# wq2012/SpectralCluster

Measured on AMD Instinct MI355X. Metric: predict() calls/sec, n=8192 d=256 ICASSP2018 (GraphCut, eigengap k in [2,20], cosine k-means), higher is better.
Workload: dtype f64; 1 GPU; icassp2018_graphcut_n8192_d256_k8_max20; n_samples=8192, n_features=256, parallelism=replicas x1, collectives=none

## Files before the change

### include/spectralcluster_amd.h

```cpp
#ifndef SPECTRALCLUSTER_AMD_H_
#define SPECTRALCLUSTER_AMD_H_

#include <stddef.h>
#include <stdint.h>

#ifdef __cplusplus
extern "C" {
#endif

#define SC_ABI_VERSION 8
#define SC_MAX_OPS 16
#define SC_MAX_BLUR_RADIUS 32
#define SC_MAX_EIG 128
#define SC_MAX_STAGES 16

typedef struct sc_handle_s* sc_handle;

typedef enum sc_status {
  SC_OK = 0,
  SC_ERR_INVALID = -1,
  SC_ERR_OOM = -2,
  SC_ERR_HIP = -3,
  SC_ERR_NOT_CONVERGED = -4,
  SC_ERR_UNSUPPORTED = -5,
// ... 231 lines not shown
                                   const double* const* affinities, const double* const* bands,
                                   double* const* outs);
int sc_stage_diffuse_rowstats(sc_handle h, const double* a, int n, int mode, double* rowmax,
                              double* rowsum, int32_t* info);
enum {
  SC_BLOCK_ROUTE_SYM = 1,
  SC_BLOCK_ROUTE_TWO_PRODUCT = 2,
  SC_BLOCK_ROUTE_GROUPED = 4
};
int sc_stage_block_operator(sc_handle h, int count, const int32_t* ns,
                            const double* const* matrices, const double* const* cvecs,
                            const double* const* pvecs, const double* const* vs_scales,
                            const double* const* vs, double* const* ws, int route);
int sc_stage_krylov_state(sc_handle h, int32_t* info, double* q, double* t, double* g, double* c,
                          double* p);
int sc_stage_laplacian(sc_handle h, int laplacian_type, const double* in, int n,
                       double* out);
int sc_stage_sym_eig(sc_handle h, const double* m, int n, int count, int descend,
                     double* values, double* vectors, sc_diag* diag);
int sc_stage_eig(sc_handle h, const double* m, int n, int count, int descend,
                 double* values, double* vectors, sc_diag* diag);
int sc_random_state_doubles(uint32_t seed, int count, double* out);
int sc_uniform_choice(int n, double u);
int sc_host_symmetric_eig(const double* a, int m, double* values, double* vectors);
int sc_host_symmetric_eig_partial(const double* a, int m, int need, double* values,
                                  double* vectors);
int sc_host_tridiag_eigvectors(const double* d, const double* e, int n, const double* lam,
                               int k, double* vectors);
int sc_host_general_eig(const double* a, int m, int nvec, double* values_re, double* values_im,
                        double* vectors_re, double* vectors_im);
// ... 40 lines not shown
```

### spectralcluster_amd/_lib.py

```python

from __future__ import annotations

import ctypes
import os
import threading
import typing

import numpy as np

SC_MAX_OPS = 16
SC_MAX_BLUR_RADIUS = 32
SC_MAX_EIG = 128
SC_MAX_STAGES = 16

SC_OK = 0
SC_ERR_INVALID = -1
SC_ERR_OOM = -2
SC_ERR_HIP = -3
SC_ERR_NOT_CONVERGED = -4
SC_ERR_UNSUPPORTED = -5
SC_ERR_NON_FINITE = -6

STAGE_NAMES = ("affinity", "refine", "diffuse", "scaling", "eig", "kmeans",
               "total", "blur", "threshold_sym", "matvec", "affinity_gemm",
# ... 127 lines not shown
    "sc_set_free_prune": (ctypes.c_int, [_handle_t, ctypes.c_int]),
    "sc_stage_diffuse_rowstats": (ctypes.c_int, [_handle_t, _c_double_p, ctypes.c_int,
                                                 ctypes.c_int, _c_double_p, _c_double_p,
                                                 ctypes.POINTER(ctypes.c_int32)]),
    "sc_stage_block_operator": (ctypes.c_int, [_handle_t, ctypes.c_int,
                                               ctypes.POINTER(ctypes.c_int32),
                                               ctypes.POINTER(_c_double_p),
                                               ctypes.POINTER(_c_double_p),
                                               ctypes.POINTER(_c_double_p),
                                               ctypes.POINTER(_c_double_p),
                                               ctypes.POINTER(_c_double_p),
                                               ctypes.POINTER(_c_double_p), ctypes.c_int]),
    "sc_stage_krylov_state": (ctypes.c_int, [_handle_t, ctypes.POINTER(ctypes.c_int32),
                                             _c_double_p, _c_double_p, _c_double_p, _c_double_p,
                                             _c_double_p]),
    "sc_config_default": (ctypes.c_int, [ctypes.POINTER(ScConfig)]),
    "sc_gaussian_weights": (ctypes.c_int, [ctypes.c_double,
                                           ctypes.POINTER(ctypes.c_int32),
                                           _c_double_p]),
    "sc_predict": (ctypes.c_int, [_handle_t, _c_double_p, ctypes.c_int, ctypes.c_int,
                                  ctypes.POINTER(ScConfig), _c_int64_p,
                                  ctypes.POINTER(ScDiag)]),
    "sc_set_embeddings": (ctypes.c_int, [_handle_t, _c_double_p, ctypes.c_int,
                                         ctypes.c_int]),
    "sc_predict_array": (ctypes.c_int, [_handle_t, ctypes.POINTER(ScArray),
                                        ctypes.POINTER(ScConfig), _c_int64_p,
                                        ctypes.POINTER(ScDiag)]),
    "sc_set_embeddings_array": (ctypes.c_int, [_handle_t, ctypes.POINTER(ScArray)]),
    "sc_predict_batch_arrays": (ctypes.c_int, [_handle_t, ctypes.POINTER(ScArray), ctypes.c_int,
                                               ctypes.POINTER(ScConfig),
# ... 336 lines not shown
```

### spectralcluster_amd/csrc/api.hip

```cpp
#include <algorithm>
#include <array>
#include <cmath>
#include <cstdio>
#include <cstdlib>
#include <cstring>
#include <vector>

#include <condition_variable>
#include <mutex>
#include <string>
#include <thread>

#include "handle.h"
#include "host_pool.h"

int ensure_matrices(sc_handle h, int n, int d, bool affinity_copy) {
  h->krylov_m = 0;
  const size_t ldn = matrix_ld(n);
  const size_t nn = (size_t)n * ldn * sizeof(double);
  if (affinity_copy) SC_TRY(grow(h, h->A0, nn));
  SC_TRY(grow(h, h->B1, nn));
  SC_TRY(grow(h, h->B2, nn));
  if (d > 0) {
    const size_t ldx = round_up(d, 16);
// ... 33 lines not shown
      SC_HIP(h, hipStreamSynchronize(h->stream));
    }
    h->tilemap_cur = ptr<int2>(h->tilemap_table) + h->tilemap_off[nt];
    return SC_OK;
  }
  if (h->tilemap_nt != nt) {
    std::vector<int2> map;
    gemm_build_sym_tilemap(nt, &map);
    SC_TRY(grow(h, h->tilemap, map.size() * sizeof(int2)));
    SC_HIP(h, hipMemcpyAsync(h->tilemap.p, map.data(), map.size() * sizeof(int2),
                             hipMemcpyHostToDevice, h->stream));
    SC_HIP(h, hipStreamSynchronize(h->stream));
    h->tilemap_nt = nt;
  }
  h->tilemap_cur = ptr<int2>(h->tilemap);
  return SC_OK;
}

int ensure_eig(sc_handle h, int n) {
  const size_t nq = (size_t)n * kLdq * sizeof(double);
  if (h->Q.bytes < nq) h->krylov_m = 0;
  SC_TRY(grow(h, h->Q, nq));
  SC_TRY(grow(h, h->Q2, nq));
  SC_TRY(grow(h, h->Vs, (size_t)n * kEigBlock * sizeof(double)));
  SC_TRY(grow(h, h->W, (size_t)n * kEigBlock * sizeof(double)));
  SC_TRY(grow(h, h->partial, std::max((size_t)kProjBlocks * kLdq * kEigBlock,
                                       lz_partial_doubles(n)) * sizeof(double)));
  SC_TRY(grow(h, h->T, (size_t)kLdq * kLdq * sizeof(double)));
  SC_TRY(grow(h, h->Y, (size_t)kLdq * kLdq * sizeof(double)));
  SC_TRY(grow(h, h->Yt, (size_t)kLdq * kLdq * sizeof(double)));
// ... 98 lines not shown
  h->pool.clear();
  for (sc_handle sub : h->gslots) sc_destroy(sub);
  h->gslots.clear();
  for (sc_handle sub : h->gshort) sc_destroy(sub);
  h->gshort.clear();
  hipSetDevice(h->device);
  hipStreamSynchronize(h->stream);
  DevBuf* bufs[] = {&h->X,     &h->Xn,    &h->A0,     &h->B1,      &h->B2,    &h->rowmax,
                    &h->rowsum, &h->cvec,  &h->pvec,   &h->tvec,    &h->deg,   &h->blurw, &h->blur_tmp, &h->dvec, &h->cut, &h->rmpart, &h->splitk, &h->tilemap, &h->tilemap_table, &h->cropval, &h->statp, &h->crvec, &h->thetai, &h->Vre, &h->Vim, &h->gpart, &h->gsrc, &h->genL, &h->ahc_size, &h->ahc_chain, &h->ahc_Z, &h->ahc_lab, &h->ahc_cent, &h->fb_part, &h->fb_small, &h->fb_x, &h->fb_cent, &h->fb_int, &h->Cq, &h->Cband, &h->cp[0], &h->cp[1], &h->cp[2], &h->cp[3], &h->cp[4], &h->symflag,
                    &h->Q,     &h->Q2,    &h->Vs,     &h->W,       &h->partial, &h->T,
                    &h->Y,     &h->Yt,    &h->theta,  &h->resid,   &h->G,     &h->Rinv,
                    &h->Hbuf,  &h->hsq,   &h->colnorm, &h->flags,  &h->E,     &h->Ek,   &h->Eio,
                    &h->td_d,  &h->td_e,  &h->td_theta, &h->td_work, &h->td_tau, &h->td_panel, &h->mvsym,
                    &h->kXc,   &h->kxsq,  &h->kclosest, &h->kcand, &h->kenorm, &h->krnd,
                    &h->kcent, &h->klab32, &h->klab64, &h->kinfo, &h->kchain, &h->gkrnd, &h->gpack, &h->gypack, &h->ginfo, &h->glabels, &h->gjtab,
                    &h->kbig, &h->kbigw, &h->fq, &h->ft32, &h->fy1, &h->fR, &h->fscal, &h->fwords, &h->fcand, &h->fY, &h->fsplit, &h->fypart, &h->frpart, &h->fq2part, &h->fmx64, &h->ftau64, &h->fplan, &h->Xalt, &h->Xstage, &h->gneg};
  for (DevBuf* b : bufs)
    if (b->p) hipFree(b->p);
  for (DevBuf& b : h->kgen)
    if (b.p) hipFree(b.p);
  for (int i = 0; i < 48; ++i) hipEventDestroy(h->ev[i]);
  if (h->h_theta) hipHostFree(h->h_theta);
  if (h->h_flags) hipHostFree(h->h_flags);
  if (h->h_rr) hipHostFree(h->h_rr);
  if (h->h_free) hipHostFree(h->h_free);
  if (h->sync_ev) hipEventDestroy(h->sync_ev);
  for (int b = 0; b < kGroupBanks; ++b) {
    if (h->gbank_ev[b]) hipEventDestroy(h->gbank_ev[b]);
    if (h->gbank_stream[b]) hipStreamDestroy(h->gbank_stream[b]);
  }
  if (h->gchain_stream) hipStreamDestroy(h->gchain_stream);
  if (h->copy_stream) hipStreamDestroy(h->copy_stream);
  if (h->gcheck_ev) hipEventDestroy(h->gcheck_ev);
  for (sc_handle lane : h->glanes) sc_destroy(lane);
  h->glanes.clear();
  delete h->gpool;
  if (h->h_gpack) hipHostFree(h->h_gpack);
  if (h->h_gypack) hipHostFree(h->h_gypack);
  if (h->h_gjtab) hipHostFree(h->h_gjtab);
  if (h->h_ginfo) hipHostFree(h->h_ginfo);
  if (h->h_glabels) hipHostFree(h->h_glabels);
  hipStreamDestroy(h->stream);
  delete h;
  return SC_OK;
}

extern "C" const char* sc_last_error(sc_handle h) { return h ? h->err.c_str() : ""; }
// ... 273 lines not shown
                     h->tilemap_cur);
      break;
    case SC_OP_ROW_WISE_NORMALIZE:
      launch_row_normalize(s, in, out, n, ld);
      break;
    default:
      return fail(h, SC_ERR_INVALID, "Unknown refinement operation");
  }
  return check_last(h, "refinement kernel launch");
}

extern "C" int sc_compute_affinity(sc_handle h) {
  if (!h) return SC_ERR_INVALID;
  if (!h->have_x) return fail(h, SC_ERR_INVALID, "no embeddings resident");
  SC_HIP(h, hipSetDevice(h->device));
  SC_TRY(ensure_tilemap(h, h->n));
  SC_TRY(grow(h, h->symflag, 16));
  SC_HIP(h, hipMemsetAsync(ptr<int>(h->symflag) + 1, 0, sizeof(int), h->stream));
  launch_normalize_rows(h->stream, ptr<double>(h->X), h->ldx, h->n, h->d,
                        ptr<double>(h->Xn), ptr<int>(h->symflag) + 1);
  h->affinity_from_embeddings = true;
  GemmRowStats rs{2, ptr<double>(h->statp), nullptr, ptr<double>(h->cropval), nullptr};
  h->aff_ev[0] = h->aff_ev[1] = -1;
  if (h->profile_level >= 1) ev_rec(h, &h->aff_ev[0]);
  launch_gemm_nt(h->stream, ptr<double>(h->Xn), h->ldx, ptr<double>(h->Xn), h->ldx,
                 ptr<double>(h->A0), h->ldn, h->n, h->n, h->d, kEpiAffinity, true,
                 ptr<double>(h->splitk), h->tilemap_cur, &rs);
  if (h->profile_level >= 1) ev_rec(h, &h->aff_ev[1]);
  SC_TRY(check_last(h, "affinity launch"));
  h->have_affinity = true;
  h->have_cropval = true;
  h->affinity_symmetric = true;
  h->constraint_applied = false;
  h->n_vec = 0;
  h->sweep_slot.clear();
  return SC_OK;
}

extern "C" int sc_set_affinity(sc_handle h, const double* a, int n) {
  if (!h) return SC_ERR_INVALID;
  if (!a || n <= 0) return fail(h, SC_ERR_INVALID, "affinity must be (n, n)");
  SC_HIP(h, hipSetDevice(h->device));
  SC_TRY(ensure_matrices(h, n, 0));
  h->n = n;
  h->ldn = matrix_ld(n);
  h->have_x = false;
  h->n_vec = 0;
  h->sweep_slot.clear();
  SC_TRY(h2d_matrix(h, a, n, n, ptr<double>(h->A0), h->ldn));
  SC_TRY(device_is_symmetric(h, ptr<double>(h->A0), n, h->ldn, &h->affinity_symmetric));
  h->have_affinity = true;
// ... 360 lines not shown
                              ptr<double>(h->Eio), ncols);
  return d2h_matrix(h, ptr<double>(h->Eio), ncols, n, ncols, out);
}

extern "C" int sc_run_resident(sc_handle h, const sc_config* cfg, int64_t* labels,
                               sc_diag* diag) {
  if (!h) return SC_ERR_INVALID;
  SC_TRY(validate_config(h, cfg));
  if (!labels) return fail(h, SC_ERR_INVALID, "labels is NULL");
  if (!h->have_x) return fail(h, SC_ERR_INVALID, "no embeddings resident");
  SC_HIP(h, hipSetDevice(h->device));
  sc_diag local;
  sc_diag* dg = diag ? diag : &local;
  memset(dg, 0, sizeof(*dg));
  h->nev = 0;
  int e0, e1, e2;
  ev_rec(h, &e0);
  SC_TRY(sc_compute_affinity(h));
  if (constraint_active(h, cfg, true)) SC_TRY(sc_apply_constraint(h, cfg));
  ev_rec(h, &e1);
  SC_TRY(eig_ncluster_impl(h, cfg, dg, nullptr, nullptr, true));
  int k = dg->n_clusters_raw;
  if (cfg->min_clusters > 0 && k < cfg->min_clusters) k = cfg->min_clusters;
  const int rc_cluster = sc_cluster(h, cfg, k, labels, dg);
  if (rc_cluster != SC_OK) {
    h->stage_events.pending = false;
    return rc_cluster;
  }
  ev_rec(h, &e2);
  SC_HIP(h, hipStreamSynchronize(h->stream));
  resolve_stage_times(h, dg);
  dg->stage_ms[SC_STAGE_AFFINITY] = ev_ms(h, e0, e1);
  dg->stage_ms[SC_STAGE_TOTAL] = ev_ms(h, e0, e2);
  if (h->profile_level >= 1)
    dg->stage_ms[SC_STAGE_AFFINITY_GEMM] = ev_ms(h, h->aff_ev[0], h->aff_ev[1]);
  return SC_OK;
}

extern "C" int sc_set_profiling(sc_handle h, int level) {
  if (!h || level < 0 || level > 2) return SC_ERR_INVALID;
  h->profile_level = level;
  return SC_OK;
}

std::vector<sc_array> host_f64_arrays(const double* const* xs, const int* ns, int d, int count) {
  std::vector<sc_array> arrays(std::max(count, 0));
  for (int i = 0; i < count; ++i) arrays[i] = host_f64_array(xs[i], ns[i], d);
  return arrays;
}

// ... 382 lines not shown
```

### spectralcluster_amd/csrc/gemm_f64.hip

```cpp
#include <algorithm>
#include <cstdio>
#include <cstdlib>
#include <type_traits>
#include <vector>

#include <cstring>

#include "sc_internal.h"

namespace sc {

typedef double v4f64 __attribute__((ext_vector_type(4)));
typedef int v4i32 __attribute__((ext_vector_type(4)));
typedef double v2f64 __attribute__((ext_vector_type(2)));

constexpr int BM = 128;
constexpr int BN = 128;
constexpr int BK = 16;

__device__ __forceinline__ int lds_chunk_off(int row, int kc) {
  return row * BK + ((2 * kc) ^ (row & 14));
}

template <bool SYM>
// ... 1016 lines not shown
    const bool self = it.B == nullptr;
    grp.m[z] = GemmPairMember{it.A, self ? it.A : it.B, it.addend, it.C, it.tilemap,
                              it.lda, self ? it.lda : it.ldb, it.ldc, it.n, nt};
    total += nt * (nt + 1) / 2;
  }
  grp.first[kGroupMax] = total;
  if (total == 0) return;
  const int xcd_chunk = (total + 7) / 8;
  const int grid = 8 * xcd_chunk;
  if (epilogue == kEpiAdd)
    hipLaunchKernelGGL((k_gemm_nt_pg<kEpiAdd>), dim3(grid), dim3(256), 0, s, grp, xcd_chunk);
  else
    hipLaunchKernelGGL((k_gemm_nt_pg<kEpiNone>), dim3(grid), dim3(256), 0, s, grp, xcd_chunk);
}

}
```

### spectralcluster_amd/csrc/handle.h

```cpp
#ifndef SPECTRALCLUSTER_AMD_HANDLE_H_
#define SPECTRALCLUSTER_AMD_HANDLE_H_

#include <algorithm>
#include <array>
#include <cmath>
#include <cstdio>
#include <cstdlib>
#include <cstring>
#include <string>
#include <vector>

#include "sc_internal.h"

using namespace sc;

struct DevBuf {
  void* p = nullptr;
  size_t bytes = 0;
};

constexpr int kKgenBufs = 12;
constexpr int kGroupBanks = 2;
constexpr int kGroupLanes = 3;

// ... 18 lines not shown
  hipStream_t copy_stream = nullptr;
  DevBuf Xstage;
  DevBuf rowmax, rowsum, cvec, pvec, tvec, deg, dvec, cut, rmpart, splitk, tilemap;
  DevBuf cropval, statp;
  DevBuf Cq, cp[5], symflag;
  DevBuf Cband;
  bool have_constraint = false, constraint_symmetric = false, constraint_applied = false;
  bool constraint_banded = false;
  bool affinity_symmetric = true;
  bool affinity_from_embeddings = false;
  int qn = 0;
  int tilemap_nt = 0;
  DevBuf tilemap_table;
  int tilemap_off[65] = {0};
  const int2* tilemap_cur = nullptr;
  DevBuf blurw;
  DevBuf blur_tmp;
  std::vector<double> blur_ext;
  DevBuf Q, Q2, Vs, W, partial, T, Y, Yt, theta, resid, G, Rinv, Hbuf, hsq, colnorm,
      flags;
  DevBuf E, Ek, Eio;
  DevBuf mvsym;
  DevBuf td_d, td_e, td_theta, td_work, td_tau, td_panel;
  std::vector<double> spectrum;
  std::vector<double> last_w;
  DevBuf crvec, thetai, Vre, Vim, gpart, gsrc, genL, gneg;
  DevBuf ahc_size, ahc_chain, ahc_Z, ahc_lab, ahc_cent;
  DevBuf fb_part, fb_small, fb_x, fb_cent, fb_int;
  DevBuf kXc, kxsq, kclosest, kcand, kenorm, krnd, kcent, klab32, klab64, kinfo, kchain;
  DevBuf kbig, kbigw;
// ... 24 lines not shown
  std::vector<int32_t> last_routes;
  int32_t* groutes = nullptr;
  std::vector<sc_handle_s*> glanes;
  class HostPool* gpool = nullptr;
  hipStream_t gbank_stream[kGroupBanks] = {nullptr};
  hipStream_t gchain_stream = nullptr;
  hipEvent_t gbank_ev[kGroupBanks] = {nullptr};
  int gconv_hist[16] = {0};
  int gconv_seen = 0;
  hipEvent_t ev[48];
  int nev = 0;
  StageEvents stage_events;
  int profile_level = 1;
  int mv_ev[16][2];
  int n_mv_ev = 0;
  int aff_ev[2] = {-1, -1};
  int blurw_radius = -1;
  double blurw_host[2 * SC_MAX_BLUR_RADIUS + 1];
  int krnd_k = -1, krnd_trials = -1;
  int kfirst_n = -1, kfirst = 0;
  int diffuse_mode = -1;
  DevBuf fq, ft32, fy1, fR, fscal, fwords, fcand, fY, fsplit, fypart, frpart;
  int free_prune = -1;
  DevBuf fq2part, fmx64, ftau64, fplan;
  int* h_free = nullptr;
  bool free_checked = false;
  int free_ev[5] = {-1, -1, -1, -1, -1};
  int krylov_m = 0, krylov_n = 0, krylov_cycles = 0, krylov_ahead = 0;
  bool krylov_free = false;
};

// ... 49 lines not shown
    b.p = nullptr;
    b.bytes = 0;
  }
  SC_HIP(h, hipMalloc(&b.p, bytes));
  b.bytes = bytes;
  return SC_OK;
}
template <typename T>
inline T* ptr(const DevBuf& b) {
  return reinterpret_cast<T*>(b.p);
}

int ensure_matrices(sc_handle h, int n, int d, bool affinity_copy = true);

int ensure_tilemap(sc_handle h, int n);
int predict_sequence(sc_handle h, const int* idx, int count, const sc_array* xs,
                     const int* ns, int d, const sc_config* cfg, int64_t* const* labels,
                     sc_diag* diags);
int validate_array(sc_handle h, const sc_array* a);
sc_array host_f64_array(const double* x, int n, int d);
std::vector<sc_array> host_f64_arrays(const double* const* xs, const int* ns, int d, int count);
bool array_is_host_f64_rows(const sc_array& a);
int ingest_embeddings(sc_handle h, const sc_array& a, bool sync, hipStream_t stream = nullptr);
int predict_batch_streams_impl(sc_handle h, const sc_array* xs, const int* ns, int d, int count,
                               const sc_config* cfg, int64_t* const* labels, sc_diag* diags,
                               int streams);
int predict_batch_grouped_impl(sc_handle h, const sc_array* xs, const int* ns, int d, int count,
                               const sc_config* cfg, int64_t* const* labels, sc_diag* diags,
                               int group);

// ... 137 lines not shown
```

### spectralcluster_amd/csrc/ingest.hip

```cpp
#include <climits>
#include <cstddef>

#include "handle.h"

namespace {

struct F16Bits { unsigned short v; };
struct BF16Bits { unsigned short v; };

__device__ __forceinline__ double widen(double v) { return v; }
__device__ __forceinline__ double widen(float v) { return (double)v; }
__device__ __forceinline__ double widen(BF16Bits b) {
  return (double)__uint_as_float((unsigned)b.v << 16);
}
__device__ __forceinline__ double widen(F16Bits b) {
  const unsigned h = b.v;
  const unsigned long long sign = (unsigned long long)(h >> 15) << 63;
  const unsigned e = (h >> 10) & 31u, m = h & 1023u;
  unsigned long long bits;
  if (e == 31u) {
    bits = sign | (0x7ffull << 52) | ((unsigned long long)m << 42);
  } else if (e != 0u) {
    bits = sign | ((unsigned long long)(e + 1008u) << 52) | ((unsigned long long)m << 42);
  } else {
// ... 108 lines not shown
  a.data = x;
  a.dtype = SC_DTYPE_F64;
  a.location = SC_MEM_HOST;
  a.rows = n;
  a.cols = d;
  a.row_stride = d;
  a.col_stride = 1;
  return a;
}

bool array_is_host_f64_rows(const sc_array& a) {
  return a.location == SC_MEM_HOST && a.dtype == SC_DTYPE_F64 && a.col_stride == 1 &&
         (a.row_stride >= a.cols || a.rows == 1);
}

int ingest_embeddings(sc_handle h, const sc_array& a, bool sync, hipStream_t stream) {
  SC_TRY(validate_array(h, &a));
  const int n = (int)a.rows, d = (int)a.cols;
  hipStream_t s = stream ? stream : h->stream;
  SC_TRY(ensure_matrices(h, n, d));
  h->n = n;
  h->d = d;
  h->ldn = matrix_ld(n);
  h->ldx = round_up(d, 16);
  h->have_affinity = h->have_cropval = false;
  h->have_x = false;
  h->n_vec = 0;
  double* X = ptr<double>(h->X);
  const size_t eb = dtype_bytes(a.dtype);
  if (a.location == SC_MEM_DEVICE) {
    launch_ingest_rows(s, a.dtype, a.data, a.row_stride, a.col_stride, n, d, X, h->ldx);
    SC_TRY(check_last(h, "ingest launch"));
  } else {
    std::vector<unsigned char> packed;
    const void* src = a.data;
    size_t spitch = (size_t)a.row_stride * eb;
    if (a.col_stride != 1 || (a.row_stride < a.cols && n > 1)) {
      pack_host_rows(a, &packed);
      src = packed.data();
      spitch = (size_t)d * eb;
      sync = true;
    }
// ... 7 lines not shown
      if (h->Xstage.bytes < need) {
        if (h->Xstage.p && s != h->stream) SC_HIP(h, hipStreamSynchronize(s));
        SC_TRY(grow(h, h->Xstage, need));
      }
      SC_HIP(h, hipMemcpy2DAsync(h->Xstage.p, pitch, src, spitch, (size_t)d * eb, n,
                                 hipMemcpyHostToDevice, s));
      launch_ingest_rows(s, a.dtype, h->Xstage.p, (long long)(pitch / eb), 1, n, d, X, h->ldx);
      SC_TRY(check_last(h, "ingest launch"));
    }
  }
  if (sync) SC_HIP(h, hipStreamSynchronize(s));
  h->have_x = true;
  return SC_OK;
}

extern "C" int sc_array_layout(int* array_bytes, int* field_offsets) {
  if (array_bytes) *array_bytes = (int)sizeof(sc_array);
  if (field_offsets) {
    field_offsets[0] = (int)offsetof(sc_array, data);
    field_offsets[1] = (int)offsetof(sc_array, dtype);
    field_offsets[2] = (int)offsetof(sc_array, location);
    field_offsets[3] = (int)offsetof(sc_array, rows);
    field_offsets[4] = (int)offsetof(sc_array, cols);
    field_offsets[5] = (int)offsetof(sc_array, row_stride);
    field_offsets[6] = (int)offsetof(sc_array, col_stride);
  }
  return SC_OK;
}

extern "C" void* sc_stream(sc_handle h) { return h ? (void*)h->stream : nullptr; }
// ... 5 lines not shown
  h->sweep_slot.clear();
  return ingest_embeddings(h, *x, true);
}

extern "C" int sc_set_embeddings(sc_handle h, const double* x, int n, int d) {
  if (!h) return SC_ERR_INVALID;
  if (!x || n <= 0 || d <= 0) return fail(h, SC_ERR_INVALID, "embeddings must be (n, d)");
  const sc_array a = host_f64_array(x, n, d);
  return sc_set_embeddings_array(h, &a);
}

extern "C" int sc_predict_array(sc_handle h, const sc_array* x, const sc_config* cfg,
                                int64_t* labels, sc_diag* diag) {
  if (!h) return SC_ERR_INVALID;
  SC_TRY(validate_config(h, cfg));
  SC_TRY(sc_set_embeddings_array(h, x));
  return sc_run_resident(h, cfg, labels, diag);
}

extern "C" int sc_predict(sc_handle h, const double* x, int n, int d, const sc_config* cfg,
                          int64_t* labels, sc_diag* diag) {
  if (!h) return SC_ERR_INVALID;
  SC_TRY(validate_config(h, cfg));
  SC_TRY(sc_set_embeddings(h, x, n, d));
  return sc_run_resident(h, cfg, labels, diag);
}

extern "C" int sc_stage_ingest(sc_handle h, const sc_array* x, double* out) {
  if (!h) return SC_ERR_INVALID;
  if (!out) return fail(h, SC_ERR_INVALID, "out is NULL");
  SC_TRY(sc_set_embeddings_array(h, x));
  return d2h_matrix(h, ptr<double>(h->X), h->ldx, h->n, h->d, out);
}

extern "C" int sc_predict_batch_arrays(sc_handle h, const sc_array* xs, int count,
                                       const sc_config* cfg, int64_t* const* labels,
                                       sc_diag* diags, int group, int streams) {
  if (!h) return SC_ERR_INVALID;
  if (!xs || !labels || count < 0) return fail(h, SC_ERR_INVALID, "NULL argument");
  SC_TRY(validate_config(h, cfg));
  SC_HIP(h, hipSetDevice(h->device));
  bool device_source = false;
  std::vector<int> ns(count);
  for (int i = 0; i < count; ++i) {
    SC_TRY(validate_array(h, xs + i));
    if (xs[i].cols != xs[0].cols)
      return fail(h, SC_ERR_INVALID, "all utterances must be (n_i, d) with the same d");
// ... 14 lines not shown
```

### spectralcluster_amd/csrc/sc_internal.h

```cpp
#pragma once

#include <hip/hip_runtime.h>

#include "switches.h"
#include <stdint.h>

#include <mutex>
#include <string>
#include <vector>

#include "../../include/spectralcluster_amd.h"

namespace sc {

constexpr int kWave = 64;
constexpr int kEigBlock = 8;
constexpr int kEigBasisCap = 128;
constexpr int kLdq = kEigBasisCap + kEigBlock;
constexpr int kDenseMax = 128;
constexpr int kHostRR = 64;
constexpr int kHostRRSingle = kEigBasisCap;
constexpr int kGenMax = 64;
constexpr int kMaxVectors = 64;
constexpr int kProjBlocks = 128;
// ... 43 lines not shown
  const double* A = nullptr;
  int lda = 0;
  const double* B = nullptr;
  int ldb = 0;
  double* C = nullptr;
  int ldc = 0;
  int n = 0;
  const int2* tilemap = nullptr;
  const double* addend = nullptr;
};
void launch_gemm_nt_pair_group(hipStream_t s, const GemmPairItem* items, int count, int epilogue);
void gemm_build_sym_tilemap(int nt, std::vector<int2>* out);
int gemm_tile_dim(int n);
int gemm_resident_slots();
size_t gemm_splitk_workspace_bytes();

void launch_normalize_rows(hipStream_t s, const double* X, int ldx, int n, int d,
                           double* Xn, int* bad_rows = nullptr);
void launch_crop_diagonal(hipStream_t s, const double* in, double* out, int n,
                          int ld);
void launch_gaussian_blur(hipStream_t s, const double* in, double* out, int n,
                          int ld, int radius, const double* weights_dev);
bool launch_gaussian_blur_fused(hipStream_t s, const double* in, double* out, int n, int ld,
                                int radius, const double* weights_dev, const double* diag,
                                double* rowmax_partials);
int blur_tile_columns(int n, int radius);
void launch_gaussian_blur_any_radius(hipStream_t s, const double* in, double* tmp, double* out,
                                     int n, int ld, int radius, const double* weights_dev);
void launch_crop_value(hipStream_t s, const double* in, int n, int ld, double* dvec);
void launch_cut_from_partials(hipStream_t s, const double* partials, int n, int ntiles,
// ... 438 lines not shown
```

### spectralcluster_amd/csrc/switches.h

```cpp
#ifndef SPECTRALCLUSTER_AMD_SWITCHES_H_
#define SPECTRALCLUSTER_AMD_SWITCHES_H_

#include <cstdlib>
#include <cstring>

namespace sc {
namespace sw {

inline int eig_trace() {
  static const int v = getenv("SC_EIG_TRACE") ? std::max(1, atoi(getenv("SC_EIG_TRACE"))) : 0;
  return v;
}
inline bool kmeans_trace() {
  static const bool v = getenv("SC_KMEANS_TRACE") != nullptr;
  return v;
}
inline bool group_trace() {
  static const bool v = getenv("SC_GROUP_TRACE") != nullptr;
  return v;
}
inline bool eig_host_chain() {
  static const bool v = getenv("SC_EIG_HOST_CHAIN") != nullptr;
  return v;
}
// ... 33 lines not shown
      getenv("SC_DIFFUSE_FREE_MIN_N") ? atoi(getenv("SC_DIFFUSE_FREE_MIN_N")) : 1536;
  return v;
}
inline int gen_dense_max_n() {
  static const int v = getenv("SC_GEN_DENSE_MAX_N") ? atoi(getenv("SC_GEN_DENSE_MAX_N")) : 512;
  return v;
}
inline bool free_no_prune() {
  static const bool v = getenv("SC_FREE_NO_PRUNE") != nullptr;
  return v;
}
inline bool sweep_one_by_one() {
  static const bool v = getenv("SC_SWEEP_ONE_BY_ONE") != nullptr;
  return v;
}

}
}

#endif
```

Before: 386.9 calls/s.

## Overlap embedding upload with paneled affinity GEMM for large inputs

For n at or above a threshold (default 7168), predict now uploads the embeddings in row panels on a copy stream. It launches the symmetric affinity GEMM piece by piece as each panel arrives, using a precomputed plan that assigns whole rounds of resident tiles to each piece. The goal is to hide the host-to-device transfer behind GEMM compute instead of running them back to back. In exchange it adds event synchronisation between streams, extra launches for the split-K tail, and plan tables built once per handle.

```diff
diff --git a/include/spectralcluster_amd.h b/include/spectralcluster_amd.h
--- a/include/spectralcluster_amd.h
+++ b/include/spectralcluster_amd.h
@@ -269,6 +269,13 @@
                             const double* const* vs, double* const* ws, int route);
 int sc_stage_krylov_state(sc_handle h, int32_t* info, double* q, double* t, double* g, double* c,
                           double* p);
+int sc_upload_panels_min_n(void);
+int sc_last_upload_panels(sc_handle h);
+int sc_upload_panel_plan(int nt, int slots, int pieces, const int32_t* end_tile_rows,
+                         const int32_t* rounds, int32_t* info, int32_t* tiles);
+int sc_stage_affinity_panels(sc_handle h, const double* x, int n, int d, int pieces,
+                             const int32_t* end_rows, const int32_t* rounds, int slots,
+                             double* affinity, double* cropval, int32_t* info);
 int sc_stage_laplacian(sc_handle h, int laplacian_type, const double* in, int n,
                        double* out);
 int sc_stage_sym_eig(sc_handle h, const double* m, int n, int count, int descend,
diff --git a/spectralcluster_amd/_lib.py b/spectralcluster_amd/_lib.py
--- a/spectralcluster_amd/_lib.py
+++ b/spectralcluster_amd/_lib.py
@@ -165,6 +165,19 @@
     "sc_stage_krylov_state": (ctypes.c_int, [_handle_t, ctypes.POINTER(ctypes.c_int32),
                                              _c_double_p, _c_double_p, _c_double_p, _c_double_p,
                                              _c_double_p]),
+    "sc_upload_panels_min_n": (ctypes.c_int, []),
+    "sc_last_upload_panels": (ctypes.c_int, [_handle_t]),
+    "sc_upload_panel_plan": (ctypes.c_int, [ctypes.c_int, ctypes.c_int, ctypes.c_int,
+                                            ctypes.POINTER(ctypes.c_int32),
+                                            ctypes.POINTER(ctypes.c_int32),
+                                            ctypes.POINTER(ctypes.c_int32),
+                                            ctypes.POINTER(ctypes.c_int32)]),
+    "sc_stage_affinity_panels": (ctypes.c_int, [_handle_t, _c_double_p, ctypes.c_int,
+                                                ctypes.c_int, ctypes.c_int,
+                                                ctypes.POINTER(ctypes.c_int32),
+                                                ctypes.POINTER(ctypes.c_int32), ctypes.c_int,
+                                                _c_double_p, _c_double_p,
+                                                ctypes.POINTER(ctypes.c_int32)]),
     "sc_config_default": (ctypes.c_int, [ctypes.POINTER(ScConfig)]),
     "sc_gaussian_weights": (ctypes.c_int, [ctypes.c_double,
                                            ctypes.POINTER(ctypes.c_int32),
diff --git a/spectralcluster_amd/csrc/api.hip b/spectralcluster_amd/csrc/api.hip
--- a/spectralcluster_amd/csrc/api.hip
+++ b/spectralcluster_amd/csrc/api.hip
@@ -71,6 +71,48 @@
     h->tilemap_nt = nt;
   }
   h->tilemap_cur = ptr<int2>(h->tilemap);
+  return SC_OK;
+}
+
+int ensure_panel_plan(sc_handle h, int n, const PanelPlan** plan, const int2** tiles) {
+  const int nt = gemm_tile_dim(n);
+  const int slots = gemm_resident_slots();
+  *plan = nullptr;
+  *tiles = nullptr;
+  if (nt < 2) return SC_OK;
+  if (nt <= kTilemapTableMax) {
+    if (!h->panel_table.p) {
+      std::vector<int2> all, one;
+      h->panel_plans.assign(kTilemapTableMax + 1, PanelPlan());
+      h->panel_off.assign(kTilemapTableMax + 1, 0);
+      for (int t = 2; t <= kTilemapTableMax; ++t) {
+        h->panel_off[t] = (int)all.size();
+        if (!gemm_default_panel_plan(t, slots, &h->panel_plans[t], &one))
+          return fail(h, SC_ERR_INVALID, "piece plan");
+        all.insert(all.end(), one.begin(), one.end());
+      }
+      SC_TRY(grow(h, h->panel_table, all.size() * sizeof(int2)));
+      SC_HIP(h, hipMemcpyAsync(h->panel_table.p, all.data(), all.size() * sizeof(int2),
+                               hipMemcpyHostToDevice, h->stream));
+      SC_HIP(h, hipStreamSynchronize(h->stream));
+    }
+    *plan = &h->panel_plans[nt];
+    *tiles = ptr<int2>(h->panel_table) + h->panel_off[nt];
+    return SC_OK;
+  }
+  if (h->panel_big_plan.nt != nt) {
+    std::vector<int2> one;
+    h->panel_big_plan = PanelPlan();
+    PanelPlan built;
+    if (!gemm_default_panel_plan(nt, slots, &built, &one)) return fail(h, SC_ERR_INVALID, "piece plan");
+    SC_TRY(grow(h, h->panel_big, one.size() * sizeof(int2)));
+    SC_HIP(h, hipMemcpyAsync(h->panel_big.p, one.data(), one.size() * sizeof(int2),
+                             hipMemcpyHostToDevice, h->stream));
+    SC_HIP(h, hipStreamSynchronize(h->stream));
+    h->panel_big_plan = built;
+  }
+  *plan = &h->panel_big_plan;
+  *tiles = ptr<int2>(h->panel_big);
   return SC_OK;
 }
 
@@ -199,7 +241,7 @@
                     &h->td_d,  &h->td_e,  &h->td_theta, &h->td_work, &h->td_tau, &h->td_panel, &h->mvsym,
                     &h->kXc,   &h->kxsq,  &h->kclosest, &h->kcand, &h->kenorm, &h->krnd,
                     &h->kcent, &h->klab32, &h->klab64, &h->kinfo, &h->kchain, &h->gkrnd, &h->gpack, &h->gypack, &h->ginfo, &h->glabels, &h->gjtab,
-                    &h->kbig, &h->kbigw, &h->fq, &h->ft32, &h->fy1, &h->fR, &h->fscal, &h->fwords, &h->fcand, &h->fY, &h->fsplit, &h->fypart, &h->frpart, &h->fq2part, &h->fmx64, &h->ftau64, &h->fplan, &h->Xalt, &h->Xstage, &h->gneg};
+                    &h->kbig, &h->kbigw, &h->fq, &h->ft32, &h->fy1, &h->fR, &h->fscal, &h->fwords, &h->fcand, &h->fY, &h->fsplit, &h->fypart, &h->frpart, &h->fq2part, &h->fmx64, &h->ftau64, &h->fplan, &h->Xalt, &h->Xstage, &h->gneg, &h->panel_table, &h->panel_big, &h->panel_own};
   for (DevBuf* b : bufs)
     if (b->p) hipFree(b->p);
   for (DevBuf& b : h->kgen)
@@ -216,6 +258,9 @@
   }
   if (h->gchain_stream) hipStreamDestroy(h->gchain_stream);
   if (h->copy_stream) hipStreamDestroy(h->copy_stream);
+  for (hipEvent_t e : h->panel_ev)
+    if (e) hipEventDestroy(e);
+  if (h->panel_idle_ev) hipEventDestroy(h->panel_idle_ev);
   if (h->gcheck_ev) hipEventDestroy(h->gcheck_ev);
   for (sc_handle lane : h->glanes) sc_destroy(lane);
   h->glanes.clear();
@@ -519,27 +564,38 @@
   if (!h) return SC_ERR_INVALID;
   if (!h->have_x) return fail(h, SC_ERR_INVALID, "no embeddings resident");
   SC_HIP(h, hipSetDevice(h->device));
-  SC_TRY(ensure_tilemap(h, h->n));
-  SC_TRY(grow(h, h->symflag, 16));
-  SC_HIP(h, hipMemsetAsync(ptr<int>(h->symflag) + 1, 0, sizeof(int), h->stream));
+  SC_TRY(affinity_begin(h, h->stream));
   launch_normalize_rows(h->stream, ptr<double>(h->X), h->ldx, h->n, h->d,
                         ptr<double>(h->Xn), ptr<int>(h->symflag) + 1);
-  h->affinity_from_embeddings = true;
   GemmRowStats rs{2, ptr<double>(h->statp), nullptr, ptr<double>(h->cropval), nullptr};
-  h->aff_ev[0] = h->aff_ev[1] = -1;
-  if (h->profile_level >= 1) ev_rec(h, &h->aff_ev[0]);
+  if (h->profile_level >= 1) ev_rec(h, &h->aff_ev[0][0]);
   launch_gemm_nt(h->stream, ptr<double>(h->Xn), h->ldx, ptr<double>(h->Xn), h->ldx,
                  ptr<double>(h->A0), h->ldn, h->n, h->n, h->d, kEpiAffinity, true,
                  ptr<double>(h->splitk), h->tilemap_cur, &rs);
-  if (h->profile_level >= 1) ev_rec(h, &h->aff_ev[1]);
+  if (h->profile_level >= 1) ev_rec(h, &h->aff_ev[0][1]);
+  h->n_aff_ev = 1;
   SC_TRY(check_last(h, "affinity launch"));
+  affinity_done(h);
+  return SC_OK;
+}
+
+int affinity_begin(sc_handle h, hipStream_t s) {
+  SC_TRY(ensure_tilemap(h, h->n));
+  SC_TRY(grow(h, h->symflag, 16));
+  SC_HIP(h, hipMemsetAsync(ptr<int>(h->symflag) + 1, 0, sizeof(int), s));
+  h->affinity_from_embeddings = true;
+  for (int k = 0; k < kMaxPanels; ++k) h->aff_ev[k][0] = h->aff_ev[k][1] = -1;
+  h->n_aff_ev = 0;
+  h->aff_paneled = false;
+  return SC_OK;
+}
+void affinity_done(sc_handle h) {
   h->have_affinity = true;
   h->have_cropval = true;
   h->affinity_symmetric = true;
   h->constraint_applied = false;
   h->n_vec = 0;
   h->sweep_slot.clear();
-  return SC_OK;
 }
 
 extern "C" int sc_set_affinity(sc_handle h, const double* a, int n) {
@@ -930,9 +986,14 @@
   sc_diag* dg = diag ? diag : &local;
   memset(dg, 0, sizeof(*dg));
   h->nev = 0;
-  int e0, e1, e2;
+  int e0;
   ev_rec(h, &e0);
   SC_TRY(sc_compute_affinity(h));
+  return run_resident_tail(h, cfg, labels, dg, e0);
+}
+
+int run_resident_tail(sc_handle h, const sc_config* cfg, int64_t* labels, sc_diag* dg, int e0) {
+  int e1, e2;
   if (constraint_active(h, cfg, true)) SC_TRY(sc_apply_constraint(h, cfg));
   ev_rec(h, &e1);
   SC_TRY(eig_ncluster_impl(h, cfg, dg, nullptr, nullptr, true));
@@ -946,10 +1007,15 @@
   ev_rec(h, &e2);
   SC_HIP(h, hipStreamSynchronize(h->stream));
   resolve_stage_times(h, dg);
-  dg->stage_ms[SC_STAGE_AFFINITY] = ev_ms(h, e0, e1);
+  float stage = ev_ms(h, e0, e1), gemm = 0.f;
+  if (h->aff_paneled && h->n_aff_ev > 0) {
+    stage = ev_ms(h, h->aff_ev[h->n_aff_ev - 1][1], e1);
+    for (int p = 0; p < h->n_aff_ev; ++p) stage += ev_ms(h, h->aff_ev[p][0], h->aff_ev[p][1]);
+  }
+  for (int p = 0; p < h->n_aff_ev; ++p) gemm += ev_ms(h, h->aff_ev[p][0], h->aff_ev[p][1]);
+  dg->stage_ms[SC_STAGE_AFFINITY] = stage;
   dg->stage_ms[SC_STAGE_TOTAL] = ev_ms(h, e0, e2);
-  if (h->profile_level >= 1)
-    dg->stage_ms[SC_STAGE_AFFINITY_GEMM] = ev_ms(h, h->aff_ev[0], h->aff_ev[1]);
+  if (h->profile_level >= 1) dg->stage_ms[SC_STAGE_AFFINITY_GEMM] = gemm;
   return SC_OK;
 }
 
diff --git a/spectralcluster_amd/csrc/gemm_f64.hip b/spectralcluster_amd/csrc/gemm_f64.hip
--- a/spectralcluster_amd/csrc/gemm_f64.hip
+++ b/spectralcluster_amd/csrc/gemm_f64.hip
@@ -1054,4 +1054,128 @@
     hipLaunchKernelGGL((k_gemm_nt_pg<kEpiNone>), dim3(grid), dim3(256), 0, s, grp, xcd_chunk);
 }
 
-}
+bool gemm_build_panel_plan(int nt, int slots, int pieces, const int* end_tile_rows,
+                           const int* rounds, PanelPlan* plan, std::vector<int2>* tiles) {
+  if (nt <= 0 || slots <= 0 || pieces < 1 || pieces > kMaxPanels) return false;
+  if (end_tile_rows[pieces - 1] != nt) return false;
+  for (int k = 0; k < pieces; ++k)
+    if (end_tile_rows[k] <= (k ? end_tile_rows[k - 1] : 0)) return false;
+  std::vector<int2> map;
+  gemm_build_sym_tilemap(nt, &map);
+  const int total = (int)map.size();
+  const int tail = total % slots;
+  std::vector<char> used(total, 0);
+  tiles->clear();
+  *plan = PanelPlan();
+  plan->nt = nt;
+  plan->slots = slots;
+  plan->pieces = pieces;
+  plan->tail = tail;
+  for (int k = 0; k < pieces; ++k) {
+    const bool last = k == pieces - 1;
+    plan->end_tile_row[k] = end_tile_rows[k];
+    plan->first[k] = (int)tiles->size();
+    int avail = 0;
+    for (int t = 0; t < total - tail; ++t)
+      if (!used[t] && map[t].y < end_tile_rows[k]) ++avail;
+    int take = avail;
+    if (!last) {
+      take = avail / slots;
+      if (rounds != nullptr && rounds[k] > 0) take = std::min(take, rounds[k]);
+      take *= slots;
+    }
+    plan->whole[k] = take;
+    for (int t = 0; t < total - tail && take > 0; ++t)
+      if (!used[t] && map[t].y < end_tile_rows[k]) {
+        tiles->push_back(map[t]);
+        used[t] = 1;
+        --take;
+      }
+    if (last) tiles->insert(tiles->end(), map.end() - tail, map.end());
+  }
+  plan->first[pieces] = (int)tiles->size();
+  return true;
+}
+
+constexpr int kPanelRoundRows = 16;
+bool gemm_default_panel_plan(int nt, int slots, PanelPlan* plan, std::vector<int2>* tiles) {
+  if (nt < 2 || slots <= 0) return false;
+  std::vector<int2> map;
+  gemm_build_sym_tilemap(nt, &map);
+  const int total = (int)map.size();
+  const int tail = total % slots;
+  std::vector<long long> cnt(nt + 1, 0);
+  for (int t = 0; t < total - tail; ++t) ++cnt[map[t].y + 1];
+  for (int b = 1; b <= nt; ++b) cnt[b] += cnt[b - 1];
+  int ends[kMaxPanels], rounds[kMaxPanels];
+  int pieces = 0;
+  long long done = 0;
+  double free_at = 0.0;
+  int b = 0;
+  while (pieces < kMaxPanels - 1) {
+    int nb = std::max(b + 1, (int)free_at);
+    while (nb < nt && cnt[nb] - done < slots) ++nb;
+    if (nb >= nt) break;
+    const int r = (int)((cnt[nb] - done) / slots);
+    while (cnt[nb - 1] - done >= (long long)r * slots) --nb;
+    ends[pieces] = nb;
+    rounds[pieces] = r;
+    done += (long long)r * slots;
+    free_at = std::max(free_at, (double)nb) + (double)r * kPanelRoundRows;
+    b = nb;
+    ++pieces;
+  }
+  if (pieces == 0) {
+    ends[0] = nt - 1;
+    rounds[0] = 0;
+    pieces = 1;
+  }
+  ends[pieces] = nt;
+  rounds[pieces] = 0;
+  ++pieces;
+  return gemm_build_panel_plan(nt, slots, pieces, ends, rounds, plan, tiles);
+}
+
+int gemm_tail_ksplit(int tiles, int tail, int slots, int K, bool have_ws) {
+  if (tail <= 0 || !have_ws) return 1;
+  const int ktiles = (K + BK - 1) / BK;
+  int ksplit = std::min(slots / tail, std::max(1, ktiles / 8));
+  if (K <= 512 && tiles - tail == 0) ksplit = 1;
+  return std::max(ksplit, 1);
+}
+
+void launch_affinity_piece(hipStream_t s, const double* Xn, int ldx, double* C, int ldc, int n,
+                           int K, double* splitk_ws, const int2* tiles, int whole, int tail,
+                           int ksplit, bool last, const GemmRowStats* rs) {
+  GemmStats stats{rs->partial_max, rs->partial_sum, rs->mode, nullptr};
+  const int tm = (n + BM - 1) / BM;
+  if (ksplit < 2) {
+    whole += tail;
+    tail = 0;
+    ksplit = 1;
+  }
+  const int grid = whole + tail * ksplit;
+  if (grid > 0) {
+    const int xcd_chunk = (whole % 8 == 0 && whole >= 512) ? whole / 8 : 0;
+    hipLaunchKernelGGL((k_gemm_nt<kEpiAffinity, true>), dim3(grid), dim3(256), 0, s, Xn, ldx, Xn,
+                       ldx, C, ldc, n, n, K, tm, tm, whole, ksplit, splitk_ws, (double*)nullptr,
+                       tiles, xcd_chunk, stats, (int*)nullptr, tail * ksplit, 0);
+  }
+  if (tail > 0) {
+    hipLaunchKernelGGL((k_gemm_reduce<kEpiAffinity, true>), dim3(tail, 16), dim3(256), 0, s,
+                       splitk_ws, C, ldc, n, n, tm, tm, whole, ksplit, tiles,
+                       (const double*)nullptr);
+    hipLaunchKernelGGL((k_gemm_tail_stats<true>), dim3(tail, 2, 8), dim3(256), 0, s, C, ldc, n, n,
+                       tm, tm, whole, tiles, stats);
+  }
+  if (!last) return;
+  if (tm <= kStatMaxTiles)
+    hipLaunchKernelGGL(k_gemm_stats_reduce_lds, dim3((n + kStatRows - 1) / kStatRows), dim3(256),
+                       2 * kStatRows * (size_t)(tm + 1) * sizeof(double), s, stats.pmax,
+                       stats.psum, n, tm, stats.mode, rs->rowmax, rs->rowsum);
+  else
+    hipLaunchKernelGGL(k_gemm_stats_reduce, dim3((n + 255) / 256), dim3(256), 0, s, stats.pmax,
+                       stats.psum, n, tm, stats.mode, rs->rowmax, rs->rowsum);
+}
+
+}
diff --git a/spectralcluster_amd/csrc/handle.h b/spectralcluster_amd/csrc/handle.h
--- a/spectralcluster_amd/csrc/handle.h
+++ b/spectralcluster_amd/csrc/handle.h
@@ -56,6 +56,12 @@
   DevBuf tilemap_table;
   int tilemap_off[65] = {0};
   const int2* tilemap_cur = nullptr;
+  DevBuf panel_table, panel_big, panel_own;
+  std::vector<PanelPlan> panel_plans;
+  std::vector<int> panel_off;
+  PanelPlan panel_big_plan;
+  hipEvent_t panel_ev[kMaxPanels] = {nullptr};
+  hipEvent_t panel_idle_ev = nullptr;
   DevBuf blurw;
   DevBuf blur_tmp;
   std::vector<double> blur_ext;
@@ -110,7 +116,9 @@
   int profile_level = 1;
   int mv_ev[16][2];
   int n_mv_ev = 0;
-  int aff_ev[2] = {-1, -1};
+  int aff_ev[kMaxPanels][2];
+  int n_aff_ev = 0;
+  bool aff_paneled = false;
   int blurw_radius = -1;
   double blurw_host[2 * SC_MAX_BLUR_RADIUS + 1];
   int krnd_k = -1, krnd_trials = -1;
@@ -190,6 +198,10 @@
 int ensure_matrices(sc_handle h, int n, int d, bool affinity_copy = true);
 
 int ensure_tilemap(sc_handle h, int n);
+int ensure_panel_plan(sc_handle h, int n, const PanelPlan** plan, const int2** tiles);
+int run_resident_tail(sc_handle h, const sc_config* cfg, int64_t* labels, sc_diag* dg, int e0);
+int affinity_begin(sc_handle h, hipStream_t s);
+void affinity_done(sc_handle h);
 int predict_sequence(sc_handle h, const int* idx, int count, const sc_array* xs,
                      const int* ns, int d, const sc_config* cfg, int64_t* const* labels,
                      sc_diag* diags);
diff --git a/spectralcluster_amd/csrc/ingest.hip b/spectralcluster_amd/csrc/ingest.hip
--- a/spectralcluster_amd/csrc/ingest.hip
+++ b/spectralcluster_amd/csrc/ingest.hip
@@ -146,10 +146,7 @@
          (a.row_stride >= a.cols || a.rows == 1);
 }
 
-int ingest_embeddings(sc_handle h, const sc_array& a, bool sync, hipStream_t stream) {
-  SC_TRY(validate_array(h, &a));
-  const int n = (int)a.rows, d = (int)a.cols;
-  hipStream_t s = stream ? stream : h->stream;
+static int begin_problem(sc_handle h, int n, int d) {
   SC_TRY(ensure_matrices(h, n, d));
   h->n = n;
   h->d = d;
@@ -158,6 +155,14 @@
   h->have_affinity = h->have_cropval = false;
   h->have_x = false;
   h->n_vec = 0;
+  return SC_OK;
+}
+
+int ingest_embeddings(sc_handle h, const sc_array& a, bool sync, hipStream_t stream) {
+  SC_TRY(validate_array(h, &a));
+  const int n = (int)a.rows, d = (int)a.cols;
+  hipStream_t s = stream ? stream : h->stream;
+  SC_TRY(begin_problem(h, n, d));
   double* X = ptr<double>(h->X);
   const size_t eb = dtype_bytes(a.dtype);
   if (a.location == SC_MEM_DEVICE) {
@@ -195,6 +200,90 @@
   return SC_OK;
 }
 
+static int paneled_front(sc_handle h, const sc_array& a, const PanelPlan& plan,
+                         const int2* tiles) {
+  const int n = (int)a.rows, d = (int)a.cols;
+  if (!h->copy_stream)
+    SC_HIP(h, hipStreamCreateWithFlags(&h->copy_stream, hipStreamNonBlocking));
+  for (int k = 0; k < plan.pieces; ++k)
+    if (!h->panel_ev[k])
+      SC_HIP(h, hipEventCreateWithFlags(&h->panel_ev[k], hipEventDisableTiming));
+  if (!h->panel_idle_ev)
+    SC_HIP(h, hipEventCreateWithFlags(&h->panel_idle_ev, hipEventDisableTiming));
+  const bool busy = hipStreamQuery(h->stream) != hipSuccess;
+  (void)hipGetLastError();
+  if (busy) {
+    SC_HIP(h, hipEventRecord(h->panel_idle_ev, h->stream));
+    SC_HIP(h, hipStreamWaitEvent(h->copy_stream, h->panel_idle_ev, 0));
+  }
+  SC_TRY(affinity_begin(h, h->copy_stream));
+  const int total = plan.nt * (plan.nt + 1) / 2;
+  const int ksplit = gemm_tail_ksplit(total, plan.tail, plan.slots, d, h->splitk.p != nullptr);
+  GemmRowStats rs{2, ptr<double>(h->statp), nullptr, ptr<double>(h->cropval), nullptr};
+  double* X = ptr<double>(h->X);
+  double* Xn = ptr<double>(h->Xn);
+  const size_t spitch = (size_t)(n == 1 ? d : a.row_stride) * sizeof(double);
+  auto enqueue = [&]() -> int {
+    for (int k = 0; k < plan.pieces; ++k) {
+      const int r0 = k ? plan.end_tile_row[k - 1] * 128 : 0;
+      const int r1 = std::min(n, plan.end_tile_row[k] * 128);
+      SC_HIP(h, hipMemcpy2DAsync(X + (size_t)r0 * h->ldx, (size_t)h->ldx * sizeof(double),
+                                 static_cast<const double*>(a.data) + (size_t)r0 * a.row_stride,
+                                 spitch, (size_t)d * sizeof(double), r1 - r0,
+                                 hipMemcpyHostToDevice, h->copy_stream));
+      launch_normalize_rows(h->copy_stream, X + (size_t)r0 * h->ldx, h->ldx, r1 - r0, d,
+                            Xn + (size_t)r0 * h->ldx, ptr<int>(h->symflag) + 1);
+      SC_HIP(h, hipEventRecord(h->panel_ev[k], h->copy_stream));
+      SC_HIP(h, hipStreamWaitEvent(h->stream, h->panel_ev[k], 0));
+      ev_rec(h, &h->aff_ev[k][0]);
+      launch_affinity_piece(h->stream, Xn, h->ldx, ptr<double>(h->A0), h->ldn, n, d,
+                            ptr<double>(h->splitk), tiles + plan.first[k], plan.whole[k],
+                            k == plan.pieces - 1 ? plan.tail : 0, ksplit, k == plan.pieces - 1,
+                            &rs);
+      ev_rec(h, &h->aff_ev[k][1]);
+      h->n_aff_ev = k + 1;
+    }
+    return check_last(h, "paneled affinity launch");
+  };
+  h->aff_paneled = true;
+  const int rc = enqueue();
+  if (rc != SC_OK) {
+    (void)hipStreamSynchronize(h->copy_stream);
+    (void)hipStreamSynchronize(h->stream);
+    return rc;
+  }
+  h->have_x = true;
+  affinity_done(h);
+  return SC_OK;
+}
+
+static bool paneled_wanted(const sc_array& a) {
+  return sw::upload_panels() && array_is_host_f64_rows(a) &&
+         a.rows >= sw::upload_panels_min_n() && gemm_tile_dim((int)a.rows) >= 2;
+}
+
+static int predict_paneled(sc_handle h, const sc_array& a, const sc_config* cfg, int64_t* labels,
+                           sc_diag* diag) {
+  if (!labels) return fail(h, SC_ERR_INVALID, "labels is NULL");
+  SC_HIP(h, hipSetDevice(h->device));
+  h->sweep_slot.clear();
+  SC_TRY(begin_problem(h, (int)a.rows, (int)a.cols));
+  const PanelPlan* plan = nullptr;
+  const int2* tiles = nullptr;
+  SC_TRY(ensure_panel_plan(h, h->n, &plan, &tiles));
+  sc_diag local;
+  sc_diag* dg = diag ? diag : &local;
+  memset(dg, 0, sizeof(*dg));
+  h->nev = 0;
+  SC_TRY(paneled_front(h, a, *plan, tiles));
+  const int rc = run_resident_tail(h, cfg, labels, dg, h->aff_ev[0][0]);
+  if (rc != SC_OK) {
+    (void)hipStreamSynchronize(h->copy_stream);
+    (void)hipStreamSynchronize(h->stream);
+  }
+  return rc;
+}
+
 extern "C" int sc_array_layout(int* array_bytes, int* field_offsets) {
   if (array_bytes) *array_bytes = (int)sizeof(sc_array);
   if (field_offsets) {
@@ -230,6 +319,8 @@
                                 int64_t* labels, sc_diag* diag) {
   if (!h) return SC_ERR_INVALID;
   SC_TRY(validate_config(h, cfg));
+  SC_TRY(validate_array(h, x));
+  if (paneled_wanted(*x)) return predict_paneled(h, *x, cfg, labels, diag);
   SC_TRY(sc_set_embeddings_array(h, x));
   return sc_run_resident(h, cfg, labels, diag);
 }
@@ -238,8 +329,9 @@
                           int64_t* labels, sc_diag* diag) {
   if (!h) return SC_ERR_INVALID;
   SC_TRY(validate_config(h, cfg));
-  SC_TRY(sc_set_embeddings(h, x, n, d));
-  return sc_run_resident(h, cfg, labels, diag);
+  if (!x || n <= 0 || d <= 0) return fail(h, SC_ERR_INVALID, "embeddings must be (n, d)");
+  const sc_array a = host_f64_array(x, n, d);
+  return sc_predict_array(h, &a, cfg, labels, diag);
 }
 
 extern "C" int sc_stage_ingest(sc_handle h, const sc_array* x, double* out) {
@@ -247,6 +339,99 @@
   if (!out) return fail(h, SC_ERR_INVALID, "out is NULL");
   SC_TRY(sc_set_embeddings_array(h, x));
   return d2h_matrix(h, ptr<double>(h->X), h->ldx, h->n, h->d, out);
+}
+
+extern "C" int sc_upload_panels_min_n(void) { return sw::upload_panels_min_n(); }
+extern "C" int sc_last_upload_panels(sc_handle h) {
+  return h && h->aff_paneled ? h->n_aff_ev : 0;
+}
+
+static void report_plan(const PanelPlan& plan, int32_t* info) {
+  info[0] = plan.pieces;
+  info[1] = plan.tail;
+  for (int k = 0; k < kMaxPanels; ++k) {
+    info[2 + k] = k < plan.pieces ? plan.end_tile_row[k] : 0;
+    info[2 + kMaxPanels + k] = k < plan.pieces ? plan.whole[k] : 0;
+  }
+}
+
+extern "C" int sc_upload_panel_plan(int nt, int slots, int pieces, const int32_t* end_tile_rows,
+                                    const int32_t* rounds, int32_t* info, int32_t* tiles) {
+  if (!info || nt < 2 || slots <= 0 || pieces < 0 || pieces > kMaxPanels) return SC_ERR_INVALID;
+  if (pieces > 0 && !end_tile_rows) return SC_ERR_INVALID;
+  PanelPlan plan;
+  std::vector<int2> list;
+  const bool ok = pieces == 0 ? gemm_default_panel_plan(nt, slots, &plan, &list)
+                              : gemm_build_panel_plan(nt, slots, pieces, end_tile_rows, rounds,
+                                                      &plan, &list);
+  if (!ok) return SC_ERR_INVALID;
+  report_plan(plan, info);
+  if (tiles)
+    for (size_t t = 0; t < list.size(); ++t) {
+      tiles[2 * t] = list[t].x;
+      tiles[2 * t + 1] = list[t].y;
+    }
+  return SC_OK;
+}
+
+extern "C" int sc_stage_affinity_panels(sc_handle h, const double* x, int n, int d, int pieces,
+                                        const int32_t* end_rows, const int32_t* rounds, int slots,
+                                        double* affinity, double* cropval, int32_t* info) {
+  if (!h) return SC_ERR_INVALID;
+  if (!x || n <= 0 || d <= 0) return fail(h, SC_ERR_INVALID, "embeddings must be (n, d)");
+  if (!affinity || !cropval || !info) return fail(h, SC_ERR_INVALID, "NULL argument");
+  SC_HIP(h, hipSetDevice(h->device));
+  const int nt = gemm_tile_dim(n);
+  if (nt < 2) return fail(h, SC_ERR_INVALID, "sc_stage_affinity_panels: one tile row has no panels");
+  if (slots < 0 || slots > gemm_resident_slots() || pieces < 0 || pieces > kMaxPanels ||
+      (pieces > 0 && !end_rows))
+    return fail(h, SC_ERR_INVALID, "sc_stage_affinity_panels: pieces or slots out of range");
+  h->sweep_slot.clear();
+  SC_TRY(begin_problem(h, n, d));
+  const PanelPlan* plan = nullptr;
+  const int2* tiles = nullptr;
+  PanelPlan own;
+  if (pieces == 0 && slots == 0) {
+    SC_TRY(ensure_panel_plan(h, n, &plan, &tiles));
+  } else {
+    int ends[kMaxPanels];
+    for (int k = 0; k < pieces; ++k) {
+      const bool last = k == pieces - 1;
+      if (last ? end_rows[k] != n : (end_rows[k] <= 0 || end_rows[k] % 128 != 0))
+        return fail(h, SC_ERR_INVALID,
+                    "sc_stage_affinity_panels: panels end at multiples of 128 rows, the last at n");
+      ends[k] = last ? nt : end_rows[k] / 128;
+    }
+    std::vector<int2> list;
+    const int g = slots > 0 ? slots : gemm_resident_slots();
+    const bool ok = pieces == 0 ? gemm_default_panel_plan(nt, g, &own, &list)
+                                : gemm_build_panel_plan(nt, g, pieces, ends, rounds, &own, &list);
+    if (!ok) return fail(h, SC_ERR_INVALID, "sc_stage_affinity_panels: the panels do not partition the rows");
+    SC_TRY(grow(h, h->panel_own, list.size() * sizeof(int2)));
+    SC_HIP(h, hipMemcpyAsync(h->panel_own.p, list.data(), list.size() * sizeof(int2),
+                             hipMemcpyHostToDevice, h->stream));
+    SC_HIP(h, hipStreamSynchronize(h->stream));
+    plan = &own;
+    tiles = ptr<int2>(h->panel_own);
+  }
+  const size_t xb = (size_t)n * h->ldx * sizeof(double);
+  SC_HIP(h, hipMemsetAsync(h->X.p, 0xff, xb, h->stream));
+  SC_HIP(h, hipMemsetAsync(h->Xn.p, 0xff, xb, h->stream));
+  SC_HIP(h, hipMemsetAsync(h->A0.p, 0xff, (size_t)n * h->ldn * sizeof(double), h->stream));
+  SC_HIP(h, hipMemsetAsync(h->cropval.p, 0xff, (size_t)n * sizeof(double), h->stream));
+  SC_HIP(h, hipMemsetAsync(h->statp.p, 0xff, (size_t)n * nt * sizeof(double), h->stream));
+  h->nev = 0;
+  const sc_array a = host_f64_array(x, n, d);
+  SC_TRY(paneled_front(h, a, *plan, tiles));
+  report_plan(*plan, info);
+  const int ksplit = gemm_tail_ksplit(nt * (nt + 1) / 2, plan->tail, plan->slots, d, true);
+  if (ksplit < 2) {
+    info[1] = 0;
+    info[2 + kMaxPanels + plan->pieces - 1] += plan->tail;
+  }
+  SC_HIP(h, hipMemcpyAsync(cropval, h->cropval.p, (size_t)n * sizeof(double),
+                           hipMemcpyDeviceToHost, h->stream));
+  return d2h_matrix(h, ptr<double>(h->A0), h->ldn, n, n, affinity);
 }
 
 extern "C" int sc_predict_batch_arrays(sc_handle h, const sc_array* xs, int count,
diff --git a/spectralcluster_amd/csrc/sc_internal.h b/spectralcluster_amd/csrc/sc_internal.h
--- a/spectralcluster_amd/csrc/sc_internal.h
+++ b/spectralcluster_amd/csrc/sc_internal.h
@@ -81,6 +81,20 @@
 int gemm_tile_dim(int n);
 int gemm_resident_slots();
 size_t gemm_splitk_workspace_bytes();
+constexpr int kMaxPanels = 4;
+struct PanelPlan {
+  int nt = 0, slots = 0, pieces = 0, tail = 0;
+  int end_tile_row[kMaxPanels] = {0};
+  int first[kMaxPanels + 1] = {0};
+  int whole[kMaxPanels] = {0};
+};
+bool gemm_build_panel_plan(int nt, int slots, int pieces, const int* end_tile_rows,
+                           const int* rounds, PanelPlan* plan, std::vector<int2>* tiles);
+bool gemm_default_panel_plan(int nt, int slots, PanelPlan* plan, std::vector<int2>* tiles);
+int gemm_tail_ksplit(int tiles, int tail, int slots, int K, bool have_ws);
+void launch_affinity_piece(hipStream_t s, const double* Xn, int ldx, double* C, int ldc, int n,
+                           int K, double* splitk_ws, const int2* tiles, int whole, int tail,
+                           int ksplit, bool last, const GemmRowStats* rs);
 
 void launch_normalize_rows(hipStream_t s, const double* X, int ldx, int n, int d,
                            double* Xn, int* bad_rows = nullptr);
diff --git a/spectralcluster_amd/csrc/switches.h b/spectralcluster_amd/csrc/switches.h
--- a/spectralcluster_amd/csrc/switches.h
+++ b/spectralcluster_amd/csrc/switches.h
@@ -71,6 +71,15 @@
   static const bool v = getenv("SC_SWEEP_ONE_BY_ONE") != nullptr;
   return v;
 }
+inline bool upload_panels() {
+  static const bool v = !(getenv("SC_UPLOAD_PANELS") && atoi(getenv("SC_UPLOAD_PANELS")) == 0);
+  return v;
+}
+inline int upload_panels_min_n() {
+  static const int v =
+      getenv("SC_UPLOAD_PANELS_MIN_N") ? atoi(getenv("SC_UPLOAD_PANELS_MIN_N")) : 7168;
+  return v;
+}
 
 }
 }
```

Result: no change. 395.5 calls/s (median of 6 runs) (+2.2%).
